# vtuber-plan/vcvits

Hardware: AMD Instinct MI355X
Metric: training utterances/sec (gen+disc step) at base.json segment_size (higher is better)
Workload: dtype f32; 1 GPU; configs/base.json widths, HiFi-GAN generator + MPD(8 periods+S) + MSD + STFT/mel-L1, G step + D step + AdamW (learning rate 0: weights held at their seeded initial values); per_gpu_batch=16, global_batch=16, segment_size=16384, parallelism=dp1, process_group_ranks=1, graph_recording_steps_before_warmup=3

## Files before the change

include/vcvits_hip.h:

```cpp
#ifndef VCVITS_HIP_H
#define VCVITS_HIP_H

#include <stdint.h>

#ifdef __cplusplus
extern "C" {
#endif

#define VCV_OK 0
#define VCV_EINVAL (-1)
#define VCV_EHIP (-2)
#define VCV_ELDS (-3)

#define VCV_ACT_NONE 0
#define VCV_ACT_LEAKY 1
#define VCV_ACT_RELU 2
#define VCV_ACT_TANH 3
#define VCV_ACT_LOGCLAMP 4

#define VCV_TF_NONE 0
#define VCV_TF_LEAKY 1
#define VCV_TF_DLEAKY 2
#define VCV_TF_DRELU 3
#define VCV_TF_DTANH 4
// ... 64 lines not shown
int vcv_conv_x3_plan(const VcvConvArgs* args, int flip, int64_t* out);
int vcv_conv_x3_run(const VcvConvArgs* args, float* pack_ws, float* scratch_ws, int flip, int pack_valid, void* stream);
int vcv_conv_x3_set_terms(int n);
int vcv_conv_x3_get_terms(void);
int vcv_conv_x3_set_all(int all);
int vcv_conv_x3_set_variant(int variant, int js, int ks);

typedef struct VcvWgradArgs {
  const float* a;
  const float* b;
  const float* aaux;
  const float* baux;
  float* dw;
  int32_t B, G, Cg, Mg;
  int32_t Ta, Tb, P;
  int32_t K;
  int32_t s, dj, off;
  int32_t a_tf, b_tf;
  int32_t transpose_out;
  float alpha, slope;
  float* dbias;
  float* slab;
  int64_t slab_floats;
} VcvWgradArgs;

int vcv_conv_wgrad(const VcvWgradArgs* args, void* stream);
int vcv_conv_wgrad_takes_dma(const VcvWgradArgs* args);

int64_t vcv_wgrad_bf16_scratch(const VcvWgradArgs* args);
int vcv_wgrad_bf16(const VcvWgradArgs* args, float* scratch, int64_t scratch_floats, void* stream);
int64_t vcv_wgrad_x3_scratch(const VcvWgradArgs* args);
int vcv_wgrad_x3(const VcvWgradArgs* args, float* scratch, int64_t scratch_floats, void* stream);
int vcv_wgrad_bf16_set_force(int cand, int z);

int vcv_conv_m1_fwd(const float* x, const float* w, const float* bias, float* y, int B, int C, int Tin,
                    int Tout, int P, int K, int stride, int dil, int pad, int in_leaky, int out_act,
                    float slope, void* stream);
int vcv_conv_c1_fwd(const float* x, const float* w, const float* bias, float* y, int B, int M, int Tin, int Tout,
                    int P, int K, int stride, int dil, int pad, int out_act, float slope, void* stream);
int vcv_conv_c1_fwd_masked(const float* x, const float* w, const float* bias, float* y, const float* oaux, int B, int M,
                           int Tin, int Tout, int P, int K, int stride, int dil, int pad, int out_act, float slope,
                           void* stream);
int vcv_conv_c1_fwd_flip(const float* x, const float* w, const float* bias, float* y, const float* oaux, int B, int M, int Tin,
                         int Tout, int P, int K, int stride, int dil, int pad, int out_act, float slope, int flip_taps,
                         void* stream);
int vcv_conv_c1_dgrad(const float* dy, const float* w, float* dx, int B, int M, int Tin, int Tout, int P, int K,
                      int stride, int dil, int pad, void* stream);
int vcv_linear_t1_fwd(const float* x, const float* w, const float* bias, float* y, int B, int C, int M, void* stream);
int vcv_linear_t1_dgrad(const float* dy, const float* w, float* dx, int B, int C, int M, void* stream);
int vcv_linear_t1_wgrad(const float* dy, const float* x, float* dw, int B, int C, int M, void* stream);
int vcv_thin_wgrad(const float* a, const float* bsh, const float* aaux, const float* baux, float* dw, int B,
                   int M, int C, int Ta, int Tb, int P, int K, int s, int d, int off, int a_tf, int b_tf,
                   float slope, float alpha, void* stream);

int vcv_grouped41_fwd(const float* x, const float* w, const float* bias, float* y, int B, int G, int Mg, int Tin,
                      int Tout, int out_act, float slope, void* stream);
int vcv_grouped41_fwd_bf16(const float* x, const float* w, const float* bias, float* y, int B, int G, int Mg, int Tin, int Tout,
                           int out_act, float slope, void* stream);
int vcv_grouped41_dgrad(const float* dy, const float* yaux, const float* w, float* dx, int B, int G, int Mg, int Tin,
                        int Tout, int dtf, float slope, void* stream);
int vcv_grouped41_dgrad_bf16(const float* dy, const float* yaux, const float* w, float* dx, int B, int G, int Mg, int Tin, int Tout,
                             int dtf, float slope, void* stream);
int vcv_grouped41_wgrad(const float* dy, const float* yaux, const float* x, float* dw, int B, int G, int Mg, int Tin,
                        int Tout, int dtf, float slope, void* stream);
int vcv_grouped41_wgrad_bf16(const float* dy, const float* yaux, const float* x, float* dw, int B, int G, int Mg, int Tin, int Tout,
                             int dtf, float slope, void* stream);
// ... 187 lines not shown
```

vcvits_amd/_lib.py:

```python
import ctypes
import os

import torch

_HERE = os.path.dirname(os.path.abspath(__file__))
from . import tuning

LIB_PATH = tuning.text("VCVITS_HIP_LIB", "", "path of another build of libvcvits_hip.so (A/B builds)") or \
    os.path.join(_HERE, "csrc", "libvcvits_hip.so")

VCV_OK = 0
ACT_NONE, ACT_LEAKY, ACT_RELU, ACT_TANH, ACT_LOGCLAMP = 0, 1, 2, 3, 4
TF_NONE, TF_LEAKY, TF_DLEAKY, TF_DRELU, TF_DTANH, TF_DLOGCLAMP = 0, 1, 2, 3, 4, 5

_f32p = ctypes.c_void_p
_i32 = ctypes.c_int32


class VcvConvArgs(ctypes.Structure):
    _fields_ = [
        ("x", _f32p), ("w", _f32p), ("bias", _f32p), ("res", _f32p), ("mask", _f32p),
        ("xaux", _f32p), ("oaux", _f32p), ("y", _f32p),
        ("B", _i32), ("G", _i32), ("Cg", _i32), ("Mg", _i32),
        ("Tin", _i32), ("Tout", _i32), ("P", _i32),
# ... 41 lines not shown
def lib():
    global _lib
    if _lib is None:
        if not os.path.exists(LIB_PATH):
            raise RuntimeError(
                "libvcvits_hip.so not found at %s -- run `python -m vcvits_amd.build_ext` "
                "(there is no CPU fallback for the vcvits hot path)" % LIB_PATH)
        L = ctypes.CDLL(LIB_PATH)
        L.vcv_version.restype = ctypes.c_char_p
        for name in EXPORTS:
            fn = getattr(L, name)
            if name != "vcv_version":
                fn.restype = (ctypes.c_int64 if name in ("vcv_conv_dma_workspace", "vcv_wgrad_bf16_scratch", "vcv_wgrad_x3_scratch", "vcv_layernorm_c_bwd_scratch", "vcv_resblock_pair_supported")
                              else ctypes.c_void_p if name == "vcv_get_seed_offset_ptr" else ctypes.c_int)
                fn.argtypes = _ARGTYPES[name]
        _lib = L
    return _lib


EXPORTS = [
    "vcv_version", "vcv_conv_gemm", "vcv_conv_wgrad", "vcv_conv_wgrad_takes_dma", "vcv_bias_grad",
    "vcv_weight_norm_fwd", "vcv_weight_norm_bwd", "vcv_spectral_norm_fwd", "vcv_spectral_norm_bwd", "vcv_avg3", "vcv_scale", "vcv_mask_mul",
    "vcv_reflect_pad_fwd", "vcv_reflect_pad_bwd", "vcv_avgpool4_fwd", "vcv_avgpool4_bwd",
    "vcv_loss_sum", "vcv_loss_grad", "vcv_adamw", "vcv_stft_mag_fwd", "vcv_stft_mag_bwd",
    "vcv_wn_gate_fwd", "vcv_wn_gate_bwd", "vcv_row_sum", "vcv_wn_res_skip_fwd", "vcv_wn_res_skip_bwd",
    "vcv_split_sample_fwd", "vcv_split_sample_bwd", "vcv_coupling", "vcv_layernorm_c_fwd",
    "vcv_layernorm_c_bwd", "vcv_rel_softmax_fwd", "vcv_rel_value_fwd", "vcv_rel_softmax_bwd",
    "vcv_kl_fwd", "vcv_kl_bwd", "vcv_nearest_fwd", "vcv_nearest_bwd", "vcv_nearest_raw_fwd", "vcv_nearest_raw_bwd", "vcv_slice_fwd", "vcv_slice_bwd",
    "vcv_dropout", "vcv_prof_begin", "vcv_prof_end", "vcv_prof_dump", "vcv_conv_m1_fwd", "vcv_conv_c1_fwd", "vcv_conv_c1_fwd_masked", "vcv_conv_c1_fwd_flip", "vcv_conv_c1_dgrad", "vcv_linear_t1_fwd", "vcv_linear_t1_dgrad", "vcv_linear_t1_wgrad", "vcv_thin_wgrad", "vcv_weight_flip_transpose",
    "vcv_act_grad", "vcv_act_grad_add", "vcv_weight_norm_many_fwd", "vcv_weight_norm_many_bwd", "vcv_loss_many_sum", "vcv_loss_many_grad", "vcv_conv_dma_workspace", "vcv_conv_dma", "vcv_conv_dma_plan", "vcv_conv_dma_run", "vcv_stft_complex_fwd", "vcv_istft", "vcv_grouped41_fwd", "vcv_grouped41_fwd_bf16", "vcv_grouped41_dgrad", "vcv_grouped41_dgrad_bf16", "vcv_grouped41_wgrad", "vcv_grouped41_wgrad_bf16",
    "vcv_prior_sample", "vcv_prof_bytes", "vcv_conv_bf16_plan", "vcv_conv_bf16_run", "vcv_wgrad_bf16_scratch", "vcv_wgrad_bf16", "vcv_act_grad_bias", "vcv_conv_pk_plan", "vcv_conv_pk_run",
    "vcv_conv_x3_plan", "vcv_conv_x3_run", "vcv_conv_x3_set_terms", "vcv_conv_x3_get_terms", "vcv_conv_x3_set_all", "vcv_wgrad_x3_scratch", "vcv_wgrad_x3", "vcv_rel_attn_supported", "vcv_rel_attn_fwd", "vcv_rel_attn_bwd", "vcv_rel_attn_bwd2", "vcv_set_deterministic", "vcv_get_deterministic", "vcv_prof_roof", "vcv_prof_pause", "vcv_conv_x3_pack_job", "vcv_conv_pk_pack_job", "vcv_conv_bf16_pack_job", "vcv_pack_many", "vcv_upload_table",
    "vcv_conv_bf16io_plan", "vcv_conv_bf16io_run", "vcv_cast_f32_x16", "vcv_cast_x16_f32", "vcv_conv_m1_x16_fwd",
    "vcv_prof_active", "vcv_set_seed_offset_ptr", "vcv_get_seed_offset_ptr", "vcv_pack_many_prepared", "vcv_adamw_dev", "vcv_set_words", "vcv_tuning_set", "vcv_tuning_get", "vcv_embedding_t_fwd", "vcv_embedding_t_fwd_checked", "vcv_embedding_t_bwd", "vcv_conv_x3_set_variant", "vcv_wgrad_bf16_set_force", "vcv_layernorm_c_bwd_scratch", "vcv_layernorm_c_bwd_ws", "vcv_resblock_pair_supported", "vcv_resblock_pair_pack", "vcv_resblock_pair_x16",
    "vcv_pyin_yin", "vcv_pyin_obs", "vcv_pyin_viterbi",
    "vcv_resample_table", "vcv_resample_apply", "vcv_phase_vocoder", "vcv_istft_ordered",
]


_P, _I, _L, _F, _D = ctypes.c_void_p, ctypes.c_int, ctypes.c_int64, ctypes.c_float, ctypes.c_double
_ARGTYPES = {
    "vcv_conv_gemm": [ctypes.POINTER(VcvConvArgs), _P],
    "vcv_conv_wgrad": [ctypes.POINTER(VcvWgradArgs), _P],
    "vcv_conv_wgrad_takes_dma": [ctypes.POINTER(VcvWgradArgs)],
    "vcv_bias_grad": [_P, _P, _P, _I, _I, _I, _I, _F, _I, _P],
    "vcv_weight_norm_fwd": [_P, _P, _P, _P, _I, _I, _P],
    "vcv_weight_norm_bwd": [_P, _P, _P, _P, _P, _P, _I, _I, _P],
    "vcv_spectral_norm_fwd": [_P, _P, _P, _P, _P, _P, _I, _I, _I, _F, _P],
    "vcv_spectral_norm_bwd": [_P, _P, _P, _P, _P, _P, _P, _I, _I, _P],
    "vcv_avg3": [_P, _P, _P, _P, _L, _P],
    "vcv_scale": [_P, _P, _F, _L, _P],
    "vcv_mask_mul": [_P, _P, _P, _I, _I, _I, _P],
    "vcv_reflect_pad_fwd": [_P, _P, _I, _I, _I, _P],
    "vcv_reflect_pad_bwd": [_P, _P, _I, _I, _I, _P],
    "vcv_avgpool4_fwd": [_P, _P, _I, _I, _P],
    "vcv_avgpool4_bwd": [_P, _P, _I, _I, _P],
    "vcv_loss_sum": [_P, _P, _F, _I, _F, _P, _L, _P],
    "vcv_loss_grad": [_P, _P, _F, _I, _F, _P, _P, _I, _L, _P],
    "vcv_adamw": [_P, _P, _P, _P, _L, _F, _F, _F, _F, _F, _I, _P],
    "vcv_stft_mag_fwd": [_P, _P, _P, _P, _I, _I, _I, _I, _I, _I, _F, _P],
    "vcv_stft_mag_bwd": [_P, _P, _P, _P, _P, _I, _I, _I, _I, _I, _I, _F, _P],
    "vcv_wn_gate_fwd": [_P, _P, _I, _I, _P, _I, _I, _I, _P],
    "vcv_wn_gate_bwd": [_P, _P, _I, _I, _P, _P, _I, _I, _I, _P],
    "vcv_row_sum": [_P, _P, _I, _I, _I, _I, _I, _P],
    "vcv_wn_res_skip_fwd": [_P, _P, _P, _P, _P, _P, _I, _I, _I, _I, _P],
    "vcv_wn_res_skip_bwd": [_P, _P, _P, _P, _P, _I, _I, _I, _P],
    "vcv_split_sample_fwd": [_P, _P, _P, _P, _P, _P, _I, _I, _I, _P],
# ... 35 lines not shown
    "vcv_thin_wgrad": [_P, _P, _P, _P, _P, _I, _I, _I, _I, _I, _I, _I, _I, _I, _I, _I, _I, _F, _F, _P],
    "vcv_weight_flip_transpose": [_P, _P, _I, _I, _I, _P],
    "vcv_grouped41_fwd": [_P, _P, _P, _P, _I, _I, _I, _I, _I, _I, _F, _P],
    "vcv_grouped41_fwd_bf16": [_P, _P, _P, _P, _I, _I, _I, _I, _I, _I, _F, _P],
    "vcv_grouped41_dgrad": [_P, _P, _P, _P, _I, _I, _I, _I, _I, _I, _F, _P],
    "vcv_grouped41_dgrad_bf16": [_P, _P, _P, _P, _I, _I, _I, _I, _I, _I, _F, _P],
    "vcv_grouped41_wgrad": [_P, _P, _P, _P, _I, _I, _I, _I, _I, _I, _F, _P],
    "vcv_grouped41_wgrad_bf16": [_P, _P, _P, _P, _I, _I, _I, _I, _I, _I, _F, _P],
    "vcv_act_grad": [_P, _P, _P, _I, _F, _L, _P],
    "vcv_act_grad_add": [_P, _P, _P, _P, _I, _F, _L, _P],
    "vcv_act_grad_bias": [_P, _P, _P, _P, _I, _I, _I, _I, _F, _P],
    "vcv_stft_complex_fwd": [_P, _P, _P, _P, _I, _I, _I, _I, _I, _I, _P],
    "vcv_istft": [_P, _P, _P, _P, _P, _I, _I, _I, _I, _I, _P],
    "vcv_loss_many_sum": [_P, _I, _I, _F, _I, _P, _P],
    "vcv_loss_many_grad": [_P, _I, _I, _F, _I, _P, _P, _P],
    "vcv_weight_norm_many_fwd": [_P, _I, _I, _P, _P, _P],
    "vcv_weight_norm_many_bwd": [_P, _I, _I, _P, _P],
    "vcv_conv_dma_workspace": [ctypes.POINTER(VcvConvArgs)],
    "vcv_conv_dma": [ctypes.POINTER(VcvConvArgs), _P, _I, _P],
    "vcv_conv_dma_plan": [ctypes.POINTER(VcvConvArgs), _I, ctypes.POINTER(ctypes.c_int64)],
    "vcv_conv_dma_run": [ctypes.POINTER(VcvConvArgs), _P, _P, _I, _I, _P],
    "vcv_prior_sample": [_P, _P, _P, _P, _L, _F, _P],
    "vcv_conv_bf16_plan": [ctypes.POINTER(VcvConvArgs), _I, ctypes.POINTER(ctypes.c_int64)],
    "vcv_conv_bf16_run": [ctypes.POINTER(VcvConvArgs), _P, _P, _I, _I, _P],
    "vcv_conv_pk_plan": [ctypes.POINTER(VcvConvArgs), _I, ctypes.POINTER(ctypes.c_int64)],
    "vcv_conv_pk_run": [ctypes.POINTER(VcvConvArgs), _P, _P, _I, _I, _P],
    "vcv_conv_x3_plan": [ctypes.POINTER(VcvConvArgs), _I, ctypes.POINTER(ctypes.c_int64)],
    "vcv_conv_x3_run": [ctypes.POINTER(VcvConvArgs), _P, _P, _I, _I, _P],
    "vcv_conv_x3_set_terms": [_I],
    "vcv_conv_x3_get_terms": [],
    "vcv_conv_x3_set_all": [_I],
    "vcv_conv_x3_set_variant": [_I, _I, _I],
    "vcv_wgrad_bf16_set_force": [_I, _I],
    "vcv_wgrad_bf16_scratch": [ctypes.POINTER(VcvWgradArgs)],
    "vcv_wgrad_x3_scratch": [ctypes.POINTER(VcvWgradArgs)],
    "vcv_wgrad_x3": [ctypes.POINTER(VcvWgradArgs), _P, _L, _P],
    "vcv_wgrad_bf16": [ctypes.POINTER(VcvWgradArgs), _P, _L, _P],
    "vcv_prof_begin": [_I],
    "vcv_prof_end": [ctypes.POINTER(ctypes.c_double), _I],
    "vcv_prof_dump": [ctypes.c_char_p],
    "vcv_prof_bytes": [ctypes.POINTER(ctypes.c_double), _I],
    "vcv_prof_roof": [ctypes.POINTER(ctypes.c_double), _I],
    "vcv_prof_pause": [_I],
    "vcv_conv_x3_pack_job": [ctypes.POINTER(VcvConvArgs), _I, ctypes.POINTER(VcvPackJob)],
    "vcv_conv_pk_pack_job": [ctypes.POINTER(VcvConvArgs), _I, ctypes.POINTER(VcvPackJob)],
    "vcv_conv_bf16_pack_job": [ctypes.POINTER(VcvConvArgs), _I, ctypes.POINTER(VcvPackJob)],
    "vcv_pack_many": [ctypes.POINTER(VcvPackJob), _I, _P, _P],
    "vcv_upload_table": [_P, _P, _L, _P],
    "vcv_pack_many_prepared": [ctypes.POINTER(VcvPackJob), _I, _P, _P],
    "vcv_tuning_set": [ctypes.c_char_p, _I],
    "vcv_tuning_get": [ctypes.c_char_p, ctypes.POINTER(ctypes.c_int)],
    "vcv_embedding_t_fwd": [_P, _P, _P, _I, _I, _I, _I, _P],
    "vcv_embedding_t_fwd_checked": [_P, _P, _P, _I, _I, _I, _I, _P, _P],
    "vcv_embedding_t_bwd": [_P, _P, _P, _I, _I, _I, _I, _I, _P],
    "vcv_set_words": [_P, _I, _I, _I, _I, _I, _P],
    "vcv_adamw_dev": [_P, _P, _P, _P, _L, _F, _F, _F, _F, _P, _I, _P],
    "vcv_conv_bf16io_plan": [ctypes.POINTER(VcvConvArgs), _I, ctypes.POINTER(ctypes.c_int64)],
    "vcv_conv_bf16io_run": [ctypes.POINTER(VcvConvArgs), _P, _P, _I, _I, _P],
    "vcv_prof_active": [],
    "vcv_set_seed_offset_ptr": [_P],
    "vcv_get_seed_offset_ptr": [],
    "vcv_cast_f32_x16": [_P, _P, _L, _I, _P],
    "vcv_cast_x16_f32": [_P, _P, _L, _I, _P],
    "vcv_conv_m1_x16_fwd": [_P, _I, _P, _P, _P, _I, _I, _I, _I, _I, _I, _I, _I, _I, _F, _P],
    "vcv_pyin_yin": [_P, _P, _P, _I, _I, _I, _I, _I, _I, _I, _I, _D, _P, _P, _P, _P],
    "vcv_pyin_obs": [_P, _P, _P, _I, _I, _I, _I, _P, _P, _P, _P, _I, _D, _D, _D, _D, _P, _P, _P],
# ... 132 lines not shown
```

vcvits_amd/csrc/wgrad_bf16.hip:

```cpp
#include "common.h"
#include "prof.h"

extern "C" int vcv_conv_x3_get_terms(void);
extern "C" int vcv_conv_x3_get_all(void);

namespace {

typedef __bf16 bf16x8 __attribute__((ext_vector_type(8)));
typedef __bf16 bf16x4 __attribute__((ext_vector_type(4)));
typedef short s16x4 __attribute__((ext_vector_type(4)));
typedef __attribute__((address_space(3))) s16x4* lds_s16x4;

constexpr int BU64 = 64;

struct WbGeom {
  int nmt, nct, ntg;
  int Z;
  int nchunk_u;
  int XR;
  int pa, pb;
  int a_bytes, buf_bytes;
  int a_plane, x_plane;
};

typedef __attribute__((address_space(3))) char lds_char;

__device__ __forceinline__ bf16x8 tr_pair(const lds_char* p0, const lds_char* p1) {
  const s16x4 lo = __builtin_amdgcn_ds_read_tr16_b64_v4i16((lds_s16x4)p0);
  const s16x4 hi = __builtin_amdgcn_ds_read_tr16_b64_v4i16((lds_s16x4)p1);
  typedef short s16x8 __attribute__((ext_vector_type(8)));
  const s16x8 v = __builtin_shufflevector(lo, hi, 0, 1, 2, 3, 4, 5, 6, 7);
  return __builtin_bit_cast(bf16x8, v);
}

template <int WM, int WC, int WU, int KT, int MAXT, int NT, int NP = 0, int BU = BU64>
__global__ void __launch_bounds__(64 * (WM * WC * WU + NP))
wgrad_bf16_kernel(const VcvWgradArgs p, const WbGeom tg, float* __restrict__ slab) {
  constexpr int BM = 32 * WM, BC = 32 * WC, NW = WM * WC * WU;
  constexpr int NS = NP ? NP : NW;
  constexpr int PL = NT == 1 ? 1 : 3;
  extern __shared__ __attribute__((aligned(16))) char smem[];
  const int tid = threadIdx.x, lane = tid & 63;
  const int wave = __builtin_amdgcn_readfirstlane(tid >> 6);
  const int sw = NP ? wave - NW : wave;
  const int wu = wave / (WM * WC), wmc = wave % (WM * WC);
  const int wm = wmc / WC, wc = wmc % WC;
  const int h = lane >> 5;

  const int ct = blockIdx.x % tg.nct, tgi = blockIdx.x / tg.nct;
  const int mt = blockIdx.y, z = blockIdx.z;
  const int K = p.K, Cg = p.Cg, Mg = p.Mg, P = p.P;
  const int k0 = tgi * KT;
  const int kn = K - k0 < KT ? K - k0 : KT;
  const int m0 = mt * BM, c0 = ct * BC;
  const int PA = tg.pa, PB = tg.pb;
  const int tap_lo = p.dj >= 0 ? k0 * p.dj : (k0 + kn - 1) * p.dj;

  const long long U = (long long)p.Ta * P;
  const long long TbP = (long long)p.Tb * P;
  const int total = p.B * tg.nchunk_u;

  f32x16 acc[KT];
#pragma unroll
  for (int k = 0; k < KT; ++k)
#pragma unroll
    for (int e = 0; e < 16; ++e) acc[k][e] = 0.f;

  const int nqa = BM / 32, nqb = BC / 32;
  const int ntA = nqa, ntB = nqb * (tg.XR / 64);
  const int ntask = ntA + ntB;
  const int lpq = lane >> 2, lg8 = lane & 3;
  f32x4 xr[MAXT][8];

  auto load = [&](int ch) {
    const int b = ch / tg.nchunk_u;
    const int uc0 = (ch - b * tg.nchunk_u) * BU;
    const int qa = uc0 / P;
    const int f0 = ((qa * p.s + p.off + tap_lo) * P) & ~3;
#pragma unroll
    for (int t = 0; t < MAXT; ++t) {
      const int task = sw + t * NS;
      if (task < ntask) {
        const bool isA = task < ntA;
        const int tt = isA ? task : task - ntA;
        const int nq = isA ? nqa : nqb;
        const int quad = tt % nq, pblk = tt / nq;
        const int chan0 = (isA ? m0 : c0) + quad * 32;
        const int climit = isA ? Mg : Cg;
        const long long rowlen = isA ? U : TbP;
        const float* base = isA ? p.a + (size_t)b * Mg * (size_t)U : p.b + (size_t)b * Cg * (size_t)TbP;
        const int pos0 = (isA ? uc0 : f0) + pblk * 64 + lpq * 4;
        const int rows = climit - chan0 < 32 ? climit - chan0 : 32;
        const unsigned rec = rows > 0 ? (unsigned)((long long)rows * rowlen * 4) : 0u;
        __amdgpu_buffer_rsrc_t rs = __builtin_amdgcn_make_buffer_rsrc((void*)(base + (size_t)chan0 * (size_t)rowlen), 0, (int)rec, 0x00020000);
        bool ok[4];
        const bool in_stage = !isA || lpq * 4 < BU;
#pragma unroll
        for (int j = 0; j < 4; ++j) ok[j] = in_stage && pos0 + j >= 0 && pos0 + j < rowlen;
#pragma unroll
        for (int e = 0; e < 8; ++e) {
          const unsigned voff = (unsigned)(((long long)(lg8 * 8 + e) * rowlen + pos0) * 4);
          f32x4 v = __builtin_bit_cast(f32x4, __builtin_amdgcn_raw_buffer_load_b128(rs, voff, 0, 0));
#pragma unroll
          for (int j = 0; j < 4; ++j) v[j] = ok[j] ? v[j] : 0.f;
          xr[t][e] = v;
        }
      }
    }
  };
  const bool do_bias = p.dbias != nullptr && blockIdx.x == 0 && sw >= 0 && sw < ntA;
  float bsum[8];
#pragma unroll
  for (int e = 0; e < 8; ++e) bsum[e] = 0.f;
  auto store = [&](int buf) {
    char* Ya = smem + buf * tg.buf_bytes;
    char* Xb = Ya + tg.a_bytes;
    if (do_bias) {
#pragma unroll
      for (int e = 0; e < 8; ++e) bsum[e] += (xr[0][e][0] + xr[0][e][1]) + (xr[0][e][2] + xr[0][e][3]);
    }
#pragma unroll
    for (int t = 0; t < MAXT; ++t) {
      const int task = sw + t * NS;
      if (task < ntask) {
        const bool isA = task < ntA;
        const int tt = isA ? task : task - ntA;
        const int nq = isA ? nqa : nqb;
        const int quad = tt % nq, pblk = tt / nq;
        const bool lk = isA ? p.a_tf == VCV_TF_LEAKY : p.b_tf == VCV_TF_LEAKY;
        char* img = isA ? Ya : Xb;
        const int pitch = isA ? PA : PB;
        const int plane = isA ? tg.a_plane : tg.x_plane;
        if (isA && lpq * 4 >= BU) continue;
#pragma unroll
        for (int j = 0; j < 4; ++j) {
          bf16x8 v, v1, v2;
#pragma unroll
          for (int e = 0; e < 8; ++e) {
            float f = xr[t][e][j];
            if (lk) f = fmaxf(f, f * p.slope);
            v[e] = (__bf16)f;
            if (PL == 3) {
              const float r1 = f - (float)v[e];
              v1[e] = (__bf16)r1;
              v2[e] = (__bf16)(r1 - (float)v1[e]);
            }
          }
          char* dst = img + (size_t)(pblk * 64 + lpq * 4 + j) * pitch + (quad * 4 + lg8) * 16;
          *reinterpret_cast<bf16x8*>(dst) = v;
          if (PL == 3) {
            *reinterpret_cast<bf16x8*>(dst + plane) = v1;
            *reinterpret_cast<bf16x8*>(dst + 2 * plane) = v2;
          }
        }
      }
    }
  };
  auto build_tab = [&](int ch, int buf) {
    int* tab = (int*)(smem + buf * tg.buf_bytes + tg.a_bytes + PL * tg.x_plane);
    const int tid = (int)threadIdx.x - (NP ? NW * 64 : 0);
    if (tid >= 0 && tid < BU) {
      const int b = ch / tg.nchunk_u;
      const int uc0 = (ch - b * tg.nchunk_u) * BU;
      const int qa = uc0 / P;
      const long long u = (long long)uc0 + tid;
      const int fs = (qa * p.s + p.off + tap_lo) * P;
      int t = fs - (fs & ~3);
      if (u < U) {
        const int q = (int)(u / P), pc = (int)(u - (long long)q * P);
        t += (q - qa) * p.s * P + pc;
      }
      tab[tid] = t * PB;
    }
  };

  const int li = lane & 15, lq = li >> 2, lp = li & 3, g1 = (lane >> 4) & 1;
  const int colA = ((wm * 32 + 16 * g1 + 4 * lp) * 2);
  const int colB = ((wc * 32 + 16 * g1 + 4 * lp) * 2);
  const int rowl = 8 * h + lq;

  if (NP && wave >= NW) {
    if (z < total) {
      __builtin_amdgcn_s_setprio(3);
      load(z);
      store(0);
      build_tab(z, 0);
      if (z + tg.Z < total) load(z + tg.Z);
      int bufi = 0;
      for (int ch = z; ch < total; ch += tg.Z) {
        asm volatile("s_waitcnt lgkmcnt(0)\n\ts_barrier" ::: "memory");
        if (ch + tg.Z < total) {
          store(bufi ^ 1);
          build_tab(ch + tg.Z, bufi ^ 1);
          if (ch + 2 * tg.Z < total) load(ch + 2 * tg.Z);
        }
        bufi ^= 1;
      }
      asm volatile("s_waitcnt lgkmcnt(0)\n\ts_barrier" ::: "memory");
    }
  } else if (z < total) {
    if (!NP) {
      load(z);
      store(0);
      build_tab(z, 0);
    }
    __syncthreads();
    int bufi = 0;
    for (int ch = z; ch < total; ch += tg.Z) {
      const bool more = !NP && ch + tg.Z < total;
      if (more) load(ch + tg.Z);
      const lds_char* Ya = (const lds_char*)smem + bufi * tg.buf_bytes;
      const lds_char* Xb = Ya + tg.a_bytes;
      const int* tab = (const int*)(smem + bufi * tg.buf_bytes + tg.a_bytes + PL * tg.x_plane);
      for (int i16 = wu; i16 < BU / 16; i16 += WU) {
        const int ur = i16 * 16 + rowl;
        bf16x8 a[PL];
#pragma unroll
        for (int pl = 0; pl < PL; ++pl) a[pl] = tr_pair(Ya + pl * tg.a_plane + ur * PA + colA, Ya + pl * tg.a_plane + (ur + 4) * PA + colA);
        const lds_char* x0 = Xb + tab[ur] + colB;
        const lds_char* x1 = Xb + tab[ur + 4] + colB;
#pragma unroll
        for (int k = 0; k < KT; ++k) {
          if (k < kn) {
            const int ro = ((k0 + k) * p.dj - tap_lo) * P * PB;
            bf16x8 bb[PL];
#pragma unroll
            for (int pl = 0; pl < PL; ++pl) bb[pl] = tr_pair(x0 + pl * tg.x_plane + ro, x1 + pl * tg.x_plane + ro);
            if (PL == 1) {
              acc[k] = __builtin_amdgcn_mfma_f32_32x32x16_bf16(a[0], bb[0], acc[k], 0, 0, 0);
            } else {
              if (NT == 9) {
                acc[k] = __builtin_amdgcn_mfma_f32_32x32x16_bf16(a[PL - 1], bb[PL - 1], acc[k], 0, 0, 0);
                acc[k] = __builtin_amdgcn_mfma_f32_32x32x16_bf16(a[PL / 2], bb[PL - 1], acc[k], 0, 0, 0);
                acc[k] = __builtin_amdgcn_mfma_f32_32x32x16_bf16(a[PL - 1], bb[PL / 2], acc[k], 0, 0, 0);
              }
              acc[k] = __builtin_amdgcn_mfma_f32_32x32x16_bf16(a[0], bb[PL - 1], acc[k], 0, 0, 0);
              acc[k] = __builtin_amdgcn_mfma_f32_32x32x16_bf16(a[PL - 1], bb[0], acc[k], 0, 0, 0);
              acc[k] = __builtin_amdgcn_mfma_f32_32x32x16_bf16(a[PL / 2], bb[PL / 2], acc[k], 0, 0, 0);
              acc[k] = __builtin_amdgcn_mfma_f32_32x32x16_bf16(a[0], bb[PL / 2], acc[k], 0, 0, 0);
              acc[k] = __builtin_amdgcn_mfma_f32_32x32x16_bf16(a[PL / 2], bb[0], acc[k], 0, 0, 0);
              acc[k] = __builtin_amdgcn_mfma_f32_32x32x16_bf16(a[0], bb[0], acc[k], 0, 0, 0);
            }
          }
        }
      }
      if (more) {
        store(bufi ^ 1);
        build_tab(ch + tg.Z, bufi ^ 1);
      }
      __syncthreads();
      bufi ^= 1;
    }
  }

  if (do_bias) {
#pragma unroll
    for (int e = 0; e < 8; ++e) {
// ... 132 lines not shown
        r[0] = acc[k].x; r[1] = acc[k].y; r[2] = acc[k].z; r[3] = acc[k].w;
      }
    }
  }
  __syncthreads();
  const int per = 32 * K;
  for (int idx = t; idx < MR * per; idx += 256) {
    const int r = idx / per, q = idx - r * per;
    const int cc = q / K, k = q - cc * K;
    const int mm = blockIdx.y * MR + r;
    if (mm < M && cb + cc < C) {
      float sum = red[r * P][k][cc];
#pragma unroll
      for (int p = 1; p < P; ++p) sum += red[r * P + p][k][cc];
      dw[((size_t)mm * C + cb + cc) * K + k] += alpha * sum;
    }
  }
}

template <int ZG>
void launch_finish4(const float* slab, float* dw, int M, int C, int K, int Z, float alpha, hipStream_t st) {
  const dim3 grid((unsigned)vcv_cdiv(C, 32), (unsigned)vcv_cdiv(M, 32 / ZG)), block(256);
#define WB_F4(kb) hipLaunchKernelGGL((wgrad_bf16_finish4_kernel<ZG, kb>), grid, block, 0, st, slab, dw, M, C, K, Z, alpha)
  if (K <= 1) WB_F4(1);
  else if (K <= 3) WB_F4(3);
  else if (K <= 5) WB_F4(5);
  else if (K <= 8) WB_F4(8);
  else if (K <= 11) WB_F4(11);
  else WB_F4(16);
#undef WB_F4
}

int g_force_cand = -1, g_force_z = -1;

constexpr int MAXT = 2;
constexpr int MAXT_WS = 3;

struct Cfg { int WM, WC, WU, KT; };

bool geometry(const VcvWgradArgs& a, const Cfg& c, WbGeom& g, size_t& lds, int PL = 1) {
  const int BU = PL == 1 ? BU64 : 32;
  const bool ws1 = vcv_tuning().wgrad_bf16_ws != 0;
  const bool ws = PL == 3 || ws1;
  const int NS = ws ? 4 : c.WM * c.WC * c.WU, maxt = ws ? MAXT_WS : MAXT;
  const int BM = 32 * c.WM, BC = 32 * c.WC, NW = c.WM * c.WC * c.WU;
  g.nmt = vcv_cdiv(a.Mg, BM);
  g.nct = vcv_cdiv(a.Cg, BC);
  g.ntg = vcv_cdiv(a.K, c.KT);
  const int adj = a.dj < 0 ? -a.dj : a.dj;
  const int qspan = (BU - 1) / a.P + 1;
  const int kspan = (c.KT < a.K ? c.KT : a.K) - 1;
  const int rowmax = (qspan * a.s + kspan * adj + 1) * a.P;
  g.XR = (rowmax + 3 + 63) & ~63;
  auto pitch = [](int w) { const int b = w * 2; return b >= 128 ? b + 64 : b; };
  g.pa = pitch(BM);
  g.pb = pitch(BC);
  g.a_plane = BU * g.pa;
  g.x_plane = g.XR * g.pb;
  g.a_bytes = PL * g.a_plane;
  g.buf_bytes = g.a_bytes + PL * g.x_plane + BU * 4;
  lds = 2ull * g.buf_bytes;
  const size_t red = c.WU > 1 ? (size_t)c.WM * c.WC * c.KT * 16 * 64 * 4 : 0;
  if (red > lds) lds = red;
  if (lds > VCV_LDS_LIMIT) return false;
  const int ntask = (BM / 32) + (BC / 32) * (g.XR / 64);
  if (ntask > maxt * NS) return false;
  if (PL == 3 && BU / 16 < c.WU) return false;
  const long long Uu = (long long)a.Ta * a.P;
  g.nchunk_u = (int)((Uu + BU - 1) / BU);
  return true;
}

template <int WM, int WC, int WU, int KT, int NT>
int launch(const VcvWgradArgs& a, const WbGeom& g0, size_t lds, float* scratch, int64_t scratch_floats, hipStream_t st) {
  WbGeom g = g0;
  const long long total = (long long)a.B * g.nchunk_u;
  const long long tiles = (long long)g.nmt * g.nct * g.ntg;
  const long long occ = lds * 2 <= VCV_LDS_LIMIT ? 2 : 1;
  const long long slots = 256 * occ;
  const size_t n = (size_t)a.Mg * a.Cg * a.K;
  long long Z = 1;
  double best = 1e30;
  for (long long z = 1; z <= total && z <= 512; ++z) {
    if ((size_t)z * n > (size_t)scratch_floats) break;
    const double rounds = (double)((tiles * z + slots - 1) / slots);
    const double cost = rounds * ((double)((total + z - 1) / z) + 2.0) / (double)occ + 0.02 * z;
    if (cost < best - 1e-9) best = cost, Z = z;
  }
  if (g_force_z > 0) {
    Z = g_force_z;
    while (Z > 1 && ((size_t)Z * n > (size_t)scratch_floats || Z > total)) --Z;
  }
  g.Z = (int)Z;
  void (*kern)(const VcvWgradArgs, const WbGeom, float*);
  const bool ws1 = vcv_tuning().wgrad_bf16_ws != 0;
  if constexpr (NT == 1) kern = ws1 ? wgrad_bf16_kernel<WM, WC, WU, KT, MAXT_WS, NT, 4, BU64> : wgrad_bf16_kernel<WM, WC, WU, KT, MAXT, NT>;
  else kern = wgrad_bf16_kernel<WM, WC, WU, KT, MAXT_WS, NT, 4, 32>;
  if (lds > 64 * 1024 && hipFuncSetAttribute((const void*)kern, hipFuncAttributeMaxDynamicSharedMemorySize, (int)lds) != hipSuccess)
    return VCV_EHIP;
  dim3 grid(g.nct * g.ntg, g.nmt, g.Z), block(64 * (WM * WC * WU + ((NT == 1 && !ws1) ? 0 : 4)));
  const double flops = 2.0 * a.B * a.Mg * a.Cg * a.K * a.P * (double)a.Ta;
  const int tag[12] = {a.B, NT == 1 ? 2 : 3, a.Cg, a.Mg, a.K, a.Ta, a.P, a.s, g.Z, 2, WM * 32 * 1000 + WC * 32, NT * 100 + KT};
  const double abytes = 4.0 * ((double)a.B * a.Mg * a.Ta * a.P + (double)a.B * a.Cg * a.Tb * a.P + (double)a.Mg * a.Cg * a.K);
  hipEvent_t ev0, ev1;
  vcv_prof_events(VCV_PROF_WGRAD_DMA, flops, tag, 12, &ev0, &ev1, abytes, NT * flops / VCV_PEAK_BF16_MFMA);
  VCV_LAUNCH_EV(kern, grid, block, (unsigned)lds, st, ev0, ev1, a, g, scratch);
  const bool finish_scalar = !vcv_tuning().wgrad_finish_vec;
  if (!finish_scalar && (a.Cg & 3) == 0 && ((uintptr_t)scratch & 15) == 0) {
    if (g.Z <= 4) launch_finish4<4>(scratch, a.dw, a.Mg, a.Cg, a.K, g.Z, a.alpha, st);
    else if (g.Z <= 8) launch_finish4<8>(scratch, a.dw, a.Mg, a.Cg, a.K, g.Z, a.alpha, st);
    else if (g.Z <= 16) launch_finish4<16>(scratch, a.dw, a.Mg, a.Cg, a.K, g.Z, a.alpha, st);
    else launch_finish4<32>(scratch, a.dw, a.Mg, a.Cg, a.K, g.Z, a.alpha, st);
  } else if (g.Z <= 12)
    hipLaunchKernelGGL(wgrad_bf16_finish_kernel<true>, dim3((unsigned)vcv_cdiv(a.Cg, 32), (unsigned)vcv_cdiv(a.Mg, 8)), dim3(256), 0,
                       st, (const float*)scratch, a.dw, a.Mg, a.Cg, a.K, g.Z, a.alpha);
  else
    hipLaunchKernelGGL(wgrad_bf16_finish_kernel<false>, dim3((unsigned)vcv_cdiv(a.Cg, 32), (unsigned)a.Mg), dim3(256), 0, st,
                       (const float*)scratch, a.dw, a.Mg, a.Cg, a.K, g.Z, a.alpha);
  return vcv_check_launch();
}

bool pick(const VcvWgradArgs& a, Cfg& c, WbGeom& g, size_t& lds, int PL = 1) {
  const bool tf_ok = (a.a_tf == VCV_TF_NONE || a.a_tf == VCV_TF_LEAKY) && (a.b_tf == VCV_TF_NONE || a.b_tf == VCV_TF_LEAKY) &&
                     a.slope >= 0.f && a.slope < 1.f;
  const long long U = (long long)a.Ta * a.P;
  if (a.G != 1 || !tf_ok || a.transpose_out || a.Mg < 32 || a.Cg < 16 || a.K > 16 || U * a.B < 256 || a.s < 1 || a.s > 3)
    return false;
  if (U * 4 >= (1ll << 31) || (long long)a.Tb * a.P * 4 >= (1ll << 31)) return false;
  c.KT = a.K == 1 ? 1 : a.K <= 3 ? 3 : a.K <= 5 ? 5 : (a.K == 7 || a.K == 8 || a.K >= 15) ? 8 : 6;
  if (PL == 3 && c.KT == 8) c.KT = 4;
  static const int cand[6][3] = {{4, 2, 1}, {4, 1, 2}, {2, 2, 2}, {2, 1, 4}, {1, 2, 4}, {1, 1, 8}};
  for (int i = 0; i < 6; ++i) {
    if (g_force_cand >= 0 && i != g_force_cand) continue;
    const int bm = 32 * cand[i][0], bc = 32 * cand[i][1];
    if (bm > 32 && bm > a.Mg) continue;
    if (bc > 32 && bc > ((a.Cg + 31) & ~31)) continue;
    c.WM = cand[i][0]; c.WC = cand[i][1]; c.WU = cand[i][2];
    if (geometry(a, c, g, lds, PL)) {
      if (PL == 3 && !vcv_conv_x3_get_all() && !(c.WC == 2 && (a.K == 5 || a.K >= 9))) return false;
      return true;
    }
  }
  return false;
}


int64_t scratch_want(const VcvWgradArgs* a, int PL) {
  Cfg c;
  WbGeom g;
  size_t lds;
  if (!a || !pick(*a, c, g, lds, PL)) return 0;
  const long long total = (long long)a->B * g.nchunk_u;
  const long long tiles = (long long)g.nmt * g.nct * g.ntg;
  long long z = (512 + tiles - 1) / tiles;
  if (z > total) z = total;
  if (z < 1) z = 1;
  const long long n = (long long)a->Mg * a->Cg * a->K;
  while (z > 1 && z * n > (64ll << 20)) --z;
  if (z > 512) z = 512;
  return (int64_t)(z * n);
}

#define WB_CASE(wm, wc, wu, kt) \
  if (c.WM == wm && c.WC == wc && c.WU == wu && c.KT == kt) return launch<wm, wc, wu, kt, NT>(*a, g, lds, scratch, scratch_floats, st)
#define WB_KT(wm, wc, wu)                                                                        \
  WB_CASE(wm, wc, wu, 1); WB_CASE(wm, wc, wu, 3); WB_CASE(wm, wc, wu, 5); WB_CASE(wm, wc, wu, 6); \
  if constexpr (NT == 1) { WB_CASE(wm, wc, wu, 8); } else { WB_CASE(wm, wc, wu, 4); }

template <int NT>
int run(const VcvWgradArgs* a, float* scratch, int64_t scratch_floats, void* stream) {
  Cfg c;
  WbGeom g;
  size_t lds;
  if (!a || !scratch || !pick(*a, c, g, lds, NT == 1 ? 1 : 3)) return VCV_EINVAL;
  if (scratch_floats < (int64_t)a->Mg * a->Cg * a->K) return VCV_EINVAL;
  hipStream_t st = (hipStream_t)stream;
  WB_KT(4, 2, 1);
  WB_KT(4, 1, 2);
  WB_KT(2, 2, 2);
  WB_KT(2, 1, 4);
  WB_KT(1, 2, 4);
  WB_KT(1, 1, 8);
  return VCV_EINVAL;
}

}

extern "C" int vcv_wgrad_bf16_set_force(int cand, int z) {
  g_force_cand = cand;
  g_force_z = z;
  return VCV_OK;
}

extern "C" int64_t vcv_wgrad_bf16_scratch(const VcvWgradArgs* a) { return scratch_want(a, 1); }
extern "C" int vcv_wgrad_bf16(const VcvWgradArgs* a, float* scratch, int64_t scratch_floats, void* stream) {
  return run<1>(a, scratch, scratch_floats, stream);
}

extern "C" int64_t vcv_wgrad_x3_scratch(const VcvWgradArgs* a) { return scratch_want(a, 3); }
extern "C" int vcv_wgrad_x3(const VcvWgradArgs* a, float* scratch, int64_t scratch_floats, void* stream) {
  return vcv_conv_x3_get_terms() == 6 ? run<6>(a, scratch, scratch_floats, stream) : run<9>(a, scratch, scratch_floats, stream);
}
```

Measured before the change: 243.8 utterances/s.

## Add period-windowed staging to x3 weight-gradient kernel with cost-based tile pick

Adds a windowed staging mode for the x3 (split-bf16) conv weight-gradient kernel on period-reshaped (P>1) MPD convolutions. Each stage now covers a small power-of-two slice of period columns over several time rows, possibly spanning batch boundaries, instead of a contiguous run of flattened positions. This is meant to cut wasted halo rows and out-of-range lanes when the period is large. The tile picker now scans all candidate tiles and window widths using a weighted stage-count cost instead of taking the first tile that fits. It also adds plan-inspection exports for testing, at the cost of more complex per-lane index computation and LDS table setup.

```diff
diff --git a/include/vcvits_hip.h b/include/vcvits_hip.h
--- a/include/vcvits_hip.h
+++ b/include/vcvits_hip.h
@@ -120,6 +120,9 @@
 int64_t vcv_wgrad_x3_scratch(const VcvWgradArgs* args);
 int vcv_wgrad_x3(const VcvWgradArgs* args, float* scratch, int64_t scratch_floats, void* stream);
 int vcv_wgrad_bf16_set_force(int cand, int z);
+int vcv_wgrad_x3_set_window(int pw);
+int vcv_wgrad_x3_plan(const VcvWgradArgs* args, int* info);
+int vcv_wgrad_x3_plan_stage(const VcvWgradArgs* args, int stage, int tap_group, int* a_src, int* x_src, int* tab);
 
 int vcv_conv_m1_fwd(const float* x, const float* w, const float* bias, float* y, int B, int C, int Tin,
                     int Tout, int P, int K, int stride, int dil, int pad, int in_leaky, int out_act,
diff --git a/vcvits_amd/_lib.py b/vcvits_amd/_lib.py
--- a/vcvits_amd/_lib.py
+++ b/vcvits_amd/_lib.py
@@ -97,7 +97,7 @@
     "vcv_prior_sample", "vcv_prof_bytes", "vcv_conv_bf16_plan", "vcv_conv_bf16_run", "vcv_wgrad_bf16_scratch", "vcv_wgrad_bf16", "vcv_act_grad_bias", "vcv_conv_pk_plan", "vcv_conv_pk_run",
     "vcv_conv_x3_plan", "vcv_conv_x3_run", "vcv_conv_x3_set_terms", "vcv_conv_x3_get_terms", "vcv_conv_x3_set_all", "vcv_wgrad_x3_scratch", "vcv_wgrad_x3", "vcv_rel_attn_supported", "vcv_rel_attn_fwd", "vcv_rel_attn_bwd", "vcv_rel_attn_bwd2", "vcv_set_deterministic", "vcv_get_deterministic", "vcv_prof_roof", "vcv_prof_pause", "vcv_conv_x3_pack_job", "vcv_conv_pk_pack_job", "vcv_conv_bf16_pack_job", "vcv_pack_many", "vcv_upload_table",
     "vcv_conv_bf16io_plan", "vcv_conv_bf16io_run", "vcv_cast_f32_x16", "vcv_cast_x16_f32", "vcv_conv_m1_x16_fwd",
-    "vcv_prof_active", "vcv_set_seed_offset_ptr", "vcv_get_seed_offset_ptr", "vcv_pack_many_prepared", "vcv_adamw_dev", "vcv_set_words", "vcv_tuning_set", "vcv_tuning_get", "vcv_embedding_t_fwd", "vcv_embedding_t_fwd_checked", "vcv_embedding_t_bwd", "vcv_conv_x3_set_variant", "vcv_wgrad_bf16_set_force", "vcv_layernorm_c_bwd_scratch", "vcv_layernorm_c_bwd_ws", "vcv_resblock_pair_supported", "vcv_resblock_pair_pack", "vcv_resblock_pair_x16",
+    "vcv_prof_active", "vcv_set_seed_offset_ptr", "vcv_get_seed_offset_ptr", "vcv_pack_many_prepared", "vcv_adamw_dev", "vcv_set_words", "vcv_tuning_set", "vcv_tuning_get", "vcv_embedding_t_fwd", "vcv_embedding_t_fwd_checked", "vcv_embedding_t_bwd", "vcv_conv_x3_set_variant", "vcv_wgrad_bf16_set_force", "vcv_wgrad_x3_set_window", "vcv_wgrad_x3_plan", "vcv_wgrad_x3_plan_stage", "vcv_layernorm_c_bwd_scratch", "vcv_layernorm_c_bwd_ws", "vcv_resblock_pair_supported", "vcv_resblock_pair_pack", "vcv_resblock_pair_x16",
     "vcv_pyin_yin", "vcv_pyin_obs", "vcv_pyin_viterbi",
     "vcv_resample_table", "vcv_resample_apply", "vcv_phase_vocoder", "vcv_istft_ordered",
 ]
@@ -199,6 +199,9 @@
     "vcv_conv_x3_set_all": [_I],
     "vcv_conv_x3_set_variant": [_I, _I, _I],
     "vcv_wgrad_bf16_set_force": [_I, _I],
+    "vcv_wgrad_x3_set_window": [_I],
+    "vcv_wgrad_x3_plan": [ctypes.POINTER(VcvWgradArgs), _P],
+    "vcv_wgrad_x3_plan_stage": [ctypes.POINTER(VcvWgradArgs), _I, _I, _P, _P, _P],
     "vcv_wgrad_bf16_scratch": [ctypes.POINTER(VcvWgradArgs)],
     "vcv_wgrad_x3_scratch": [ctypes.POINTER(VcvWgradArgs)],
     "vcv_wgrad_x3": [ctypes.POINTER(VcvWgradArgs), _P, _L, _P],
diff --git a/vcvits_amd/csrc/wgrad_bf16.hip b/vcvits_amd/csrc/wgrad_bf16.hip
--- a/vcvits_amd/csrc/wgrad_bf16.hip
+++ b/vcvits_amd/csrc/wgrad_bf16.hip
@@ -21,7 +21,85 @@
   int pa, pb;
   int a_bytes, buf_bytes;
   int a_plane, x_plane;
+  int total;
+  int PW, LW, QW, npc;
 };
+
+struct WbStage {
+  int b, uc0, fs;
+  int pc0, b0, q0, rem;
+};
+
+__host__ __device__ inline WbStage wb_stage(const VcvWgradArgs& p, const WbGeom& g, int BU, int tap_lo, int ch) {
+  WbStage st = {0, 0, 0, 0, 0, 0, 0};
+  if (g.PW == 0) {
+    st.b = ch / g.nchunk_u;
+    st.uc0 = (ch - st.b * g.nchunk_u) * BU;
+    st.fs = ((st.uc0 / p.P) * p.s + p.off + tap_lo) * p.P;
+  } else {
+    const int si = ch / g.npc;
+    st.pc0 = (ch - si * g.npc) << g.LW;
+    const int r0 = si * g.QW, R = p.B * p.Ta;
+    st.b0 = r0 / p.Ta;
+    st.q0 = r0 - st.b0 * p.Ta;
+    st.rem = R - r0 < g.QW ? R - r0 : g.QW;
+  }
+  return st;
+}
+
+__host__ __device__ inline bool wb_win_row(const VcvWgradArgs& p, const WbStage& st, int lo, int span, bool isA, int w, int& b, int& row,
+                                           int& xw) {
+  bool ok = false;
+  b = 0, row = 0, xw = 0;
+  int abase = 0, xbase = 0, rem = st.rem;
+  for (int bb = st.b0, q = st.q0; rem > 0; ++bb, q = 0) {
+    const int nq = rem < p.Ta - q ? rem : p.Ta - q;
+    const int xcnt = (nq - 1) * p.s + span;
+    if (isA) {
+      if (w >= abase && w < abase + nq) ok = true, b = bb, row = q + (w - abase), xw = xbase + (w - abase) * p.s;
+    } else if (w >= xbase && w < xbase + xcnt) {
+      ok = true, b = bb, row = q * p.s + lo + (w - xbase);
+    }
+    abase += nq, xbase += xcnt, rem -= nq;
+  }
+  return ok;
+}
+
+__host__ __device__ inline unsigned wb_src4(const VcvWgradArgs& p, const WbGeom& g, const WbStage& st, int BU, int lo, int span, bool isA,
+                                            int img0, int& b, int& pos0) {
+  unsigned m = 0;
+  if (g.PW == 0) {
+    const long long rowlen = (long long)(isA ? p.Ta : p.Tb) * p.P;
+    b = st.b;
+    pos0 = (isA ? st.uc0 : (st.fs & ~3)) + img0;
+    if (!isA || img0 < BU)
+      for (int j = 0; j < 4; ++j) m |= (pos0 + j >= 0 && pos0 + j < rowlen) ? 1u << j : 0u;
+  } else {
+    int row, xw;
+    const int w = img0 >> g.LW, col = st.pc0 + (img0 & (g.PW - 1));
+    bool ok = wb_win_row(p, st, lo, span, isA, w, b, row, xw);
+    ok = ok && row >= 0 && row < (isA ? p.Ta : p.Tb) && (!isA || img0 < BU);
+    pos0 = row * p.P + col;
+    if (ok)
+      for (int j = 0; j < 4; ++j) m |= col + j < p.P ? 1u << j : 0u;
+  }
+  return m;
+}
+
+__host__ __device__ inline int wb_tab(const VcvWgradArgs& p, const WbGeom& g, const WbStage& st, int lo, int span, int i) {
+  if (g.PW == 0) {
+    int t = st.fs - (st.fs & ~3);
+    const long long u = (long long)st.uc0 + i;
+    if (u < (long long)p.Ta * p.P) {
+      const int qa = st.uc0 / p.P, q = (int)(u / p.P), pc = (int)(u - (long long)q * p.P);
+      t += (q - qa) * p.s * p.P + pc;
+    }
+    return t;
+  }
+  int b, row, xw;
+  wb_win_row(p, st, lo, span, true, i >> g.LW, b, row, xw);
+  return (xw << g.LW) + (i & (g.PW - 1));
+}
 
 typedef __attribute__((address_space(3))) char lds_char;
 
@@ -58,7 +136,9 @@
 
   const long long U = (long long)p.Ta * P;
   const long long TbP = (long long)p.Tb * P;
-  const int total = p.B * tg.nchunk_u;
+  const int total = tg.total;
+  const int PWl = tg.PW ? tg.PW : P;
+  const int span = (kn - 1) * (p.dj < 0 ? -p.dj : p.dj) + 1;
 
   f32x16 acc[KT];
 #pragma unroll
@@ -67,16 +147,14 @@
     for (int e = 0; e < 16; ++e) acc[k][e] = 0.f;
 
   const int nqa = BM / 32, nqb = BC / 32;
-  const int ntA = nqa, ntB = nqb * (tg.XR / 64);
+  const int ntA = nqa, ntB = nqb * ((tg.XR + 63) / 64);
   const int ntask = ntA + ntB;
   const int lpq = lane >> 2, lg8 = lane & 3;
   f32x4 xr[MAXT][8];
 
   auto load = [&](int ch) {
-    const int b = ch / tg.nchunk_u;
-    const int uc0 = (ch - b * tg.nchunk_u) * BU;
-    const int qa = uc0 / P;
-    const int f0 = ((qa * p.s + p.off + tap_lo) * P) & ~3;
+    const WbStage stg = wb_stage(p, tg, BU, tap_lo, ch);
+    const bool win = tg.PW != 0;
 #pragma unroll
     for (int t = 0; t < MAXT; ++t) {
       const int task = sw + t * NS;
@@ -88,21 +166,24 @@
         const int chan0 = (isA ? m0 : c0) + quad * 32;
         const int climit = isA ? Mg : Cg;
         const long long rowlen = isA ? U : TbP;
-        const float* base = isA ? p.a + (size_t)b * Mg * (size_t)U : p.b + (size_t)b * Cg * (size_t)TbP;
-        const int pos0 = (isA ? uc0 : f0) + pblk * 64 + lpq * 4;
+        const int img0 = pblk * 64 + lpq * 4;
+        if (!isA && img0 >= tg.XR) continue;
+        int b, pos0;
+        const unsigned okm = wb_src4(p, tg, stg, BU, p.off + tap_lo, span, isA, img0, b, pos0);
+        const float* tbase = isA ? p.a : p.b;
         const int rows = climit - chan0 < 32 ? climit - chan0 : 32;
-        const unsigned rec = rows > 0 ? (unsigned)((long long)rows * rowlen * 4) : 0u;
-        __amdgpu_buffer_rsrc_t rs = __builtin_amdgcn_make_buffer_rsrc((void*)(base + (size_t)chan0 * (size_t)rowlen), 0, (int)rec, 0x00020000);
-        bool ok[4];
-        const bool in_stage = !isA || lpq * 4 < BU;
-#pragma unroll
-        for (int j = 0; j < 4; ++j) ok[j] = in_stage && pos0 + j >= 0 && pos0 + j < rowlen;
+        const long long recl = win ? (long long)p.B * climit * rowlen * 4 : rows > 0 ? (long long)rows * rowlen * 4 : 0;
+        const float* dbase = win ? tbase : tbase + ((size_t)stg.b * climit + chan0) * (size_t)rowlen;
+        __amdgpu_buffer_rsrc_t rs = __builtin_amdgcn_make_buffer_rsrc((void*)dbase, 0, (int)(unsigned)recl, 0x00020000);
+        const int crow = win ? b * climit + chan0 + lg8 * 8 : lg8 * 8;
+        const int nrl = win ? climit - chan0 - lg8 * 8 : 8;
 #pragma unroll
         for (int e = 0; e < 8; ++e) {
-          const unsigned voff = (unsigned)(((long long)(lg8 * 8 + e) * rowlen + pos0) * 4);
+          unsigned voff = (unsigned)(((long long)(crow + e) * rowlen + pos0) * 4);
+          if (e >= nrl) voff = 0x80000000u;
           f32x4 v = __builtin_bit_cast(f32x4, __builtin_amdgcn_raw_buffer_load_b128(rs, voff, 0, 0));
 #pragma unroll
-          for (int j = 0; j < 4; ++j) v[j] = ok[j] ? v[j] : 0.f;
+          for (int j = 0; j < 4; ++j) v[j] = (okm >> j) & 1 ? v[j] : 0.f;
           xr[t][e] = v;
         }
       }
@@ -131,7 +212,7 @@
         char* img = isA ? Ya : Xb;
         const int pitch = isA ? PA : PB;
         const int plane = isA ? tg.a_plane : tg.x_plane;
-        if (isA && lpq * 4 >= BU) continue;
+        if (isA ? lpq * 4 >= BU : pblk * 64 + lpq * 4 >= tg.XR) continue;
 #pragma unroll
         for (int j = 0; j < 4; ++j) {
           bf16x8 v, v1, v2;
@@ -159,19 +240,7 @@
   auto build_tab = [&](int ch, int buf) {
     int* tab = (int*)(smem + buf * tg.buf_bytes + tg.a_bytes + PL * tg.x_plane);
     const int tid = (int)threadIdx.x - (NP ? NW * 64 : 0);
-    if (tid >= 0 && tid < BU) {
-      const int b = ch / tg.nchunk_u;
-      const int uc0 = (ch - b * tg.nchunk_u) * BU;
-      const int qa = uc0 / P;
-      const long long u = (long long)uc0 + tid;
-      const int fs = (qa * p.s + p.off + tap_lo) * P;
-      int t = fs - (fs & ~3);
-      if (u < U) {
-        const int q = (int)(u / P), pc = (int)(u - (long long)q * P);
-        t += (q - qa) * p.s * P + pc;
-      }
-      tab[tid] = t * PB;
-    }
+    if (tid >= 0 && tid < BU) tab[tid] = wb_tab(p, tg, wb_stage(p, tg, BU, tap_lo, ch), p.off + tap_lo, span, tid) * PB;
   };
 
   const int li = lane & 15, lq = li >> 2, lp = li & 3, g1 = (lane >> 4) & 1;
@@ -222,7 +291,7 @@
 #pragma unroll
         for (int k = 0; k < KT; ++k) {
           if (k < kn) {
-            const int ro = ((k0 + k) * p.dj - tap_lo) * P * PB;
+            const int ro = ((k0 + k) * p.dj - tap_lo) * PWl * PB;
             bf16x8 bb[PL];
 #pragma unroll
             for (int pl = 0; pl < PL; ++pl) bb[pl] = tr_pair(x0 + pl * tg.x_plane + ro, x1 + pl * tg.x_plane + ro);
@@ -421,13 +490,14 @@
 }
 
 int g_force_cand = -1, g_force_z = -1;
+int g_force_win = -1;
 
 constexpr int MAXT = 2;
 constexpr int MAXT_WS = 3;
 
 struct Cfg { int WM, WC, WU, KT; };
 
-bool geometry(const VcvWgradArgs& a, const Cfg& c, WbGeom& g, size_t& lds, int PL = 1) {
+bool geometry(const VcvWgradArgs& a, const Cfg& c, WbGeom& g, size_t& lds, int PL = 1, int pw = 0) {
   const int BU = PL == 1 ? BU64 : 32;
   const bool ws1 = vcv_tuning().wgrad_bf16_ws != 0;
   const bool ws = PL == 3 || ws1;
@@ -437,10 +507,28 @@
   g.nct = vcv_cdiv(a.Cg, BC);
   g.ntg = vcv_cdiv(a.K, c.KT);
   const int adj = a.dj < 0 ? -a.dj : a.dj;
-  const int qspan = (BU - 1) / a.P + 1;
   const int kspan = (c.KT < a.K ? c.KT : a.K) - 1;
-  const int rowmax = (qspan * a.s + kspan * adj + 1) * a.P;
-  g.XR = (rowmax + 3 + 63) & ~63;
+  const long long Uu = (long long)a.Ta * a.P;
+  g.PW = pw, g.LW = 0, g.QW = 0, g.npc = 1;
+  g.nchunk_u = (int)((Uu + BU - 1) / BU);
+  if (pw == 0) {
+    const int qspan = (BU - 1) / a.P + 1;
+    const int rowmax = (qspan * a.s + kspan * adj + 1) * a.P + 3;
+    g.XR = PL == 3 ? (rowmax + 15) & ~15 : (rowmax + 63) & ~63;
+    g.total = a.B * g.nchunk_u;
+  } else {
+    if (PL != 3 || a.P <= 1 || pw < 4 || pw > BU / 2 || (pw & (pw - 1))) return false;
+    if ((long long)a.B * a.Mg * Uu * 4 >= (1ll << 31) || (long long)a.B * a.Cg * a.Tb * a.P * 4 >= (1ll << 31)) return false;
+    while ((1 << g.LW) < pw) ++g.LW;
+    g.QW = BU / pw;
+    g.npc = vcv_cdiv(a.P, pw);
+    int nseg = a.Ta % g.QW == 0 ? 1 : 1 + (g.QW - 1 + a.Ta - 1) / a.Ta;
+    if (nseg > a.B) nseg = a.B;
+    const int span = kspan * adj + 1;
+    const int xw1 = (g.QW - 1) * a.s + span, xwn = (g.QW - nseg) * a.s + nseg * span;
+    g.XR = ((xw1 > xwn ? xw1 : xwn) * pw + 15) & ~15;
+    g.total = g.npc * (int)(((long long)a.B * a.Ta + g.QW - 1) / g.QW);
+  }
   auto pitch = [](int w) { const int b = w * 2; return b >= 128 ? b + 64 : b; };
   g.pa = pitch(BM);
   g.pb = pitch(BC);
@@ -452,18 +540,16 @@
   const size_t red = c.WU > 1 ? (size_t)c.WM * c.WC * c.KT * 16 * 64 * 4 : 0;
   if (red > lds) lds = red;
   if (lds > VCV_LDS_LIMIT) return false;
-  const int ntask = (BM / 32) + (BC / 32) * (g.XR / 64);
+  const int ntask = (BM / 32) + (BC / 32) * ((g.XR + 63) / 64);
   if (ntask > maxt * NS) return false;
   if (PL == 3 && BU / 16 < c.WU) return false;
-  const long long Uu = (long long)a.Ta * a.P;
-  g.nchunk_u = (int)((Uu + BU - 1) / BU);
   return true;
 }
 
 template <int WM, int WC, int WU, int KT, int NT>
 int launch(const VcvWgradArgs& a, const WbGeom& g0, size_t lds, float* scratch, int64_t scratch_floats, hipStream_t st) {
   WbGeom g = g0;
-  const long long total = (long long)a.B * g.nchunk_u;
+  const long long total = g.total;
   const long long tiles = (long long)g.nmt * g.nct * g.ntg;
   const long long occ = lds * 2 <= VCV_LDS_LIMIT ? 2 : 1;
   const long long slots = 256 * occ;
@@ -518,19 +604,32 @@
   if (U * 4 >= (1ll << 31) || (long long)a.Tb * a.P * 4 >= (1ll << 31)) return false;
   c.KT = a.K == 1 ? 1 : a.K <= 3 ? 3 : a.K <= 5 ? 5 : (a.K == 7 || a.K == 8 || a.K >= 15) ? 8 : 6;
   if (PL == 3 && c.KT == 8) c.KT = 4;
+  c.WM = c.WC = c.WU = 0;
   static const int cand[6][3] = {{4, 2, 1}, {4, 1, 2}, {2, 2, 2}, {2, 1, 4}, {1, 2, 4}, {1, 1, 8}};
+  static const double TILE_W[6] = {1.0, 1.5, 1.05, 1.7, 1.5, 2.2};
+  static const int WINS[4] = {0, 4, 8, 16};
+  const bool plans = PL == 3 && a.P > 1;
+  double best = 1e300;
   for (int i = 0; i < 6; ++i) {
     if (g_force_cand >= 0 && i != g_force_cand) continue;
     const int bm = 32 * cand[i][0], bc = 32 * cand[i][1];
     if (bm > 32 && bm > a.Mg) continue;
     if (bc > 32 && bc > ((a.Cg + 31) & ~31)) continue;
-    c.WM = cand[i][0]; c.WC = cand[i][1]; c.WU = cand[i][2];
-    if (geometry(a, c, g, lds, PL)) {
-      if (PL == 3 && !vcv_conv_x3_get_all() && !(c.WC == 2 && (a.K == 5 || a.K >= 9))) return false;
-      return true;
-    }
-  }
-  return false;
+    Cfg ci = c;
+    ci.WM = cand[i][0]; ci.WC = cand[i][1]; ci.WU = cand[i][2];
+    for (int wi = 0; wi < (plans ? 4 : 1); ++wi) {
+      if (plans && g_force_win >= 0 && WINS[wi] != g_force_win) continue;
+      WbGeom gi;
+      size_t li;
+      if (!geometry(a, ci, gi, li, PL, WINS[wi])) continue;
+      const double cost = (double)gi.total * TILE_W[i];
+      if (cost < best) best = cost, c = ci, g = gi, lds = li;
+    }
+    if (!plans && best < 1e300) break;
+  }
+  if (best >= 1e300) return false;
+  if (PL == 3 && !vcv_conv_x3_get_all() && !(c.WC == 2 && (a.K == 5 || a.K >= 9))) return false;
+  return true;
 }
 
 
@@ -539,7 +638,7 @@
   WbGeom g;
   size_t lds;
   if (!a || !pick(*a, c, g, lds, PL)) return 0;
-  const long long total = (long long)a->B * g.nchunk_u;
+  const long long total = g.total;
   const long long tiles = (long long)g.nmt * g.nct * g.ntg;
   long long z = (512 + tiles - 1) / tiles;
   if (z > total) z = total;
@@ -581,6 +680,48 @@
   return VCV_OK;
 }
 
+extern "C" int vcv_wgrad_x3_set_window(int pw) {
+  g_force_win = pw;
+  return VCV_OK;
+}
+
+extern "C" int vcv_wgrad_x3_plan(const VcvWgradArgs* a, int* info) {
+  Cfg c;
+  WbGeom g;
+  size_t lds;
+  if (!a || !info || !pick(*a, c, g, lds, 3)) return VCV_EINVAL;
+  const int v[16] = {32 * c.WM, 32 * c.WC, c.KT, g.ntg, g.PW, g.QW, g.npc, g.total, g.XR, 32, (int)lds, g.PW ? g.PW : a->P, g.pb, 0, 0, 0};
+  for (int i = 0; i < 16; ++i) info[i] = v[i];
+  return VCV_OK;
+}
+extern "C" int vcv_wgrad_x3_plan_stage(const VcvWgradArgs* a, int stage, int tgi, int* a_src, int* x_src, int* tab) {
+  Cfg c;
+  WbGeom g;
+  size_t lds;
+  if (!a || !a_src || !x_src || !tab || !pick(*a, c, g, lds, 3)) return VCV_EINVAL;
+  if (stage < 0 || stage >= g.total || tgi < 0 || tgi >= g.ntg) return VCV_EINVAL;
+  const int BU = 32, k0 = tgi * c.KT, kn = a->K - k0 < c.KT ? a->K - k0 : c.KT;
+  const int tap_lo = a->dj >= 0 ? k0 * a->dj : (k0 + kn - 1) * a->dj;
+  const int span = (kn - 1) * (a->dj < 0 ? -a->dj : a->dj) + 1, lo = a->off + tap_lo;
+  const WbStage st = wb_stage(*a, g, BU, tap_lo, stage);
+  for (int isA = 1; isA >= 0; --isA) {
+    int* out = isA ? a_src : x_src;
+    const int rows = isA ? BU : g.XR;
+    for (int img0 = 0; img0 < rows; img0 += 4) {
+      int b, pos0;
+      const unsigned m = wb_src4(*a, g, st, BU, lo, span, isA != 0, img0, b, pos0);
+      for (int j = 0; j < 4; ++j) {
+        const bool ok = (m >> j) & 1;
+        out[(img0 + j) * 3 + 0] = ok ? b : -1;
+        out[(img0 + j) * 3 + 1] = ok ? (pos0 + j) / a->P : -1;
+        out[(img0 + j) * 3 + 2] = ok ? (pos0 + j) % a->P : -1;
+      }
+    }
+  }
+  for (int i = 0; i < BU; ++i) tab[i] = wb_tab(*a, g, st, lo, span, i);
+  return VCV_OK;
+}
+
 extern "C" int64_t vcv_wgrad_bf16_scratch(const VcvWgradArgs* a) { return scratch_want(a, 1); }
 extern "C" int vcv_wgrad_bf16(const VcvWgradArgs* a, float* scratch, int64_t scratch_floats, void* stream) {
   return run<1>(a, scratch, scratch_floats, stream);
```

Result: no change. 244.2 utterances/s, median of 6 (+0.2%).
